# honglu2875/hironaka

Measured on AMD Instinct MI355X. Metric: env-steps/sec at dim=3, max_pts=20, batch=65536; 1/2/4/8 GPUs, higher is better.
Workload: dtype f32

## Files before the change

hironaka_amd/csrc/hk_duo_kernel.h:

```cpp
#pragma once

#include "hk_fast_kernel.h"

namespace hk {

constexpr int kDuoGames = kWave / 2;

__device__ __forceinline__ int duo_other_i(int v) { return qperm_i<0xB1>(v); }
__device__ __forceinline__ float duo_other(float v) { return __int_as_float(duo_other_i(__float_as_int(v))); }

__device__ __forceinline__ uint64_t duo_ballot(bool p) { return __builtin_amdgcn_ballot_w64(p); }

template <int M, int D>
struct DuoGeom {
  using G = FastGeom<M, D>;
  static constexpr int CH = (G::C + 1) / 2;
  static constexpr int QH = (kDuoGames * G::Q + kWave - 1) / kWave;
  static constexpr bool kLean = CH * D <= 30;
};

template <int M, int D>
struct DuoSlabRegs {
  typename VecOf<FastGeom<M, D>::W>::type v[DuoGeom<M, D>::QH];
};

template <int M, int D, bool CONTIG>
__device__ __forceinline__ void duo_slab_issue_impl(DuoSlabRegs<M, D>& r, const float* base, int64_t in_stride,
                                                    int ngames, int lane) {
  using G = FastGeom<M, D>;
  using V = typename VecOf<G::W>::type;
  const int total = ngames * G::Q;
#pragma unroll
  for (int it = 0; it < DuoGeom<M, D>::QH; ++it) {
    int q = lane + it * kWave;
    q = q < total ? q : total - 1;
    r.v[it] = *reinterpret_cast<const V*>(base + slab_chunk_global<M, D, CONTIG>(q, in_stride));
  }
}

template <int M, int D>
__device__ __forceinline__ void duo_slab_issue(DuoSlabRegs<M, D>& r, const float* in, int64_t in_stride, int64_t g0,
                                               int ngames, int lane) {
  const float* base = in + g0 * in_stride;
  if (in_stride == FastGeom<M, D>::N) duo_slab_issue_impl<M, D, true>(r, base, in_stride, ngames, lane);
  else duo_slab_issue_impl<M, D, false>(r, base, in_stride, ngames, lane);
}

template <int M, int D>
__device__ __forceinline__ void duo_slab_commit(DuoSlabRegs<M, D>& r, float* lds, int ngames, int lane) {
  using G = FastGeom<M, D>;
  using V = typename VecOf<G::W>::type;
  const int total = ngames * G::Q;
#pragma unroll
  for (int it = 0; it < DuoGeom<M, D>::QH; ++it) asm volatile("" : "+v"(r.v[it]));
#pragma unroll
  for (int it = 0; it < DuoGeom<M, D>::QH; ++it) {
    const int q = lane + it * kWave;
    if (q < total) *reinterpret_cast<V*>(lds + slab_chunk_lds<M, D>(q)) = r.v[it];
  }
}

constexpr int kStorePlain = 0, kStoreNT = 1, kStoreWT = 2;

template <int M, int D, bool CONTIG, int kBatch, int ST = kStorePlain>
__device__ __forceinline__ void duo_store_slab_impl(const float* lds, float* base, int64_t out_stride, int ngames,
                                                    int lane) {
  using G = FastGeom<M, D>;
  using V = typename VecOf<G::W>::type;
  constexpr int QH = DuoGeom<M, D>::QH;
  constexpr bool kWT = ST == kStoreWT && CONTIG && G::W == 4;
  const int total = ngames * G::Q;
#pragma unroll
  for (int i0 = 0; i0 < QH; i0 += kBatch) {
    V v[kBatch];
#pragma unroll
    for (int u = 0; u < kBatch; ++u) {
      int q = lane + (i0 + u) * kWave;
      q = q < kDuoGames * G::Q ? q : kDuoGames * G::Q - 1;
      v[u] = *reinterpret_cast<const V*>(lds + slab_chunk_lds<M, D>(q));
    }
#pragma unroll
    for (int u = 0; u < kBatch; ++u) asm volatile("" : "+v"(v[u]));
    if constexpr (kWT) {
      typedef unsigned int vu4 __attribute__((ext_vector_type(4)));
      const uint64_t b = (uint64_t)base;
      const uint32_t blo = __builtin_amdgcn_readfirstlane((uint32_t)b), bhi = __builtin_amdgcn_readfirstlane((uint32_t)(b >> 32));
      const int bytes = __builtin_amdgcn_readfirstlane(total * G::W * (int)sizeof(float));
      const auto rsrc = __builtin_amdgcn_make_buffer_rsrc((void*)(((uint64_t)bhi << 32) | blo), 0, bytes, 0x00020000);
#pragma unroll
      for (int u = 0; u < kBatch; ++u) {
        const int q = lane + (i0 + u) * kWave;
        if (i0 + u < QH && q < total)
          __builtin_amdgcn_raw_buffer_store_b128(__builtin_bit_cast(vu4, v[u]), rsrc, q * G::W * (int)sizeof(float), 0,
                                                 16);
      }
    } else {
#pragma unroll
      for (int u = 0; u < kBatch; ++u) {
        const int q = lane + (i0 + u) * kWave;
        if (i0 + u < QH && q < total) {
          V* dst = reinterpret_cast<V*>(base + slab_chunk_global<M, D, CONTIG>(q, out_stride));
          if constexpr (ST != kStorePlain) __builtin_nontemporal_store(v[u], dst);
          else *dst = v[u];
        }
      }
    }
  }
}

template <int M, int D, int kBatch = DuoGeom<M, D>::QH, int ST = kStorePlain>
__device__ inline void duo_store_slab(const float* lds, float* out, int64_t out_stride, int64_t g0, int ngames,
                                      int lane) {
  float* base = out + g0 * out_stride;
  if (out_stride == FastGeom<M, D>::N) duo_store_slab_impl<M, D, true, kBatch, ST>(lds, base, out_stride, ngames, lane);
  else duo_store_slab_impl<M, D, false, kBatch, ST>(lds, base, out_stride, ngames, lane);
}

struct DuoLadder {
  static constexpr int next_bucket(int nb) { return nb < 6 ? nb + 1 : nb + 2; }
};

template <int M, int CH, int D, int SB = CH>
__device__ __forceinline__ void duo_gather_slots(float (&q)[CH * D], const float* mine, uint32_t mask, int smax, int h) {
  mask = h ? (mask & (mask - 1)) : mask;
  unrolled_while<0, SB>([&](auto sc) {
    constexpr int s = decltype(sc)::value;
    if (s >= smax) return false;
    const bool has = mask != 0;
    const float* row = mine + (has ? mask_first(mask) : 0) * D;
    mask &= mask - 1;
    mask &= mask - 1;
#pragma unroll
    for (int k = 0; k < D; ++k) {
      const float v = row[k];
      q[s * D + k] = has ? v : INFINITY;
    }
    return true;
  });
}

template <int CH, int D, int NB, int SB = NB>
__device__ __forceinline__ void duo_gather_level(float (&q)[CH * D], const float* mine, const float* hole, uint32_t mask,
                                                 int h) {
  mask = h ? (mask & (mask - 1)) : mask;
  const float* row[NB];
#pragma unroll
  for (int s = 0; s < NB; ++s) {
    row[s] = mask != 0 ? mine + mask_first(mask) * D : hole;
    mask &= mask - 1;
    mask &= mask - 1;
  }
#pragma unroll
  for (int s = 0; s < NB; ++s)
#pragma unroll
    for (int k = 0; k < D; ++k) q[s * D + k] = row[s][k];
#pragma unroll
  for (int e = NB * D; e < SB * D; ++e) q[e] = INFINITY;
}

template <int M, int CH, int D, bool LEVELS, int SB = CH>
__device__ __forceinline__ void duo_gather(float (&q)[CH * D], const float* mine, const float* hole, uint32_t mask,
                                           int smax, int h) {
  if constexpr (LEVELS) {
    StagesFor<DuoLadder, SB>::run(smax, [&](auto nb) {
      duo_gather_level<CH, D, decltype(nb)::value, SB>(q, mine, hole, mask, h);
      return 0;
    });
  } else {
    duo_gather_slots<M, CH, D, SB>(q, mine, mask, smax, h);
  }
}

template <int CH, int D, int NB>
__device__ __forceinline__ uint32_t duo_scatter_level(const float (&q)[CH * D], float* mine, uint32_t mask, int h) {
  mask = h ? (mask & (mask - 1)) : mask;
  uint32_t alive = 0;
#pragma unroll
  for (int s = 0; s < NB; ++s) {
    if (mask != 0 && q[s * D] < INFINITY) {
      const int slot = mask_first(mask);
      alive |= 1u << slot;
      float* row = mine + slot * D;
#pragma unroll
      for (int k = 0; k < D; ++k) row[k] = q[s * D + k];
    }
    mask &= mask - 1;
    mask &= mask - 1;
  }
  return alive;
}

template <int M, int CH, int D, int SB = CH>
__device__ __forceinline__ uint32_t duo_scatter(const float (&q)[CH * D], float* mine, uint32_t mask, int smax, int h) {
  mask = h ? (mask & (mask - 1)) : mask;
  uint32_t alive = 0;
  unrolled_while<0, SB>([&](auto sc) {
    constexpr int s = decltype(sc)::value;
    if (s >= smax) return false;
    if (mask != 0 && q[s * D] < INFINITY) {
      const int slot = mask_first(mask);
      alive |= 1u << slot;
      float* row = mine + slot * D;
#pragma unroll
      for (int k = 0; k < D; ++k) row[k] = q[s * D + k];
    }
    mask &= mask - 1;
    mask &= mask - 1;
    return true;
  });
  return lanes_or<2>(alive);
}

template <int D>
__device__ __forceinline__ void duo_pad_rows(float* mine, uint32_t dead, float pad, int h) {
  dead = h ? (dead & (dead - 1)) : dead;
  while (dead != 0) {
    float* row = mine + mask_first(dead) * D;
#pragma unroll
    for (int k = 0; k < D; ++k) row[k] = pad;
    dead &= dead - 1;
    dead &= dead - 1;
  }
}

template <int M, int D>
__device__ __forceinline__ void duo_scan_half(const float* mine, float fill, int h, uint32_t& live, bool& ok) {
  static_assert(M <= 32, "the game's mask is one word");
  constexpr int C = (M + 1) / 2;
  const int i0 = h * C;
  const float* base = mine + i0 * D;
  uint32_t mask = 0;
  ok = true;
  const uint32_t fill_bits = __float_as_uint(fill);
#pragma unroll
  for (int r = 0; r < C; ++r) {
    const bool valid = (M % 2 == 0) || r + 1 < C || h == 0;
    uint32_t hi = __float_as_uint(base[r * D]), lo = hi;
#pragma unroll
    for (int k = 1; k < D; ++k) {
      const uint32_t u = __float_as_uint(base[r * D + k]);
      hi = u > hi ? u : hi;
      lo = u < lo ? u : lo;
    }
    const bool ge = hi < 0x7F800000u;
    const bool fl = (lo == fill_bits) && (hi == fill_bits);
    ok &= (ge | fl | !valid);
    mask |= (ge && valid) ? (1u << r) : 0u;
  }
  mask <<= i0;
  live = lanes_or<2>(mask);
}

template <int CH, int D, int NB>
__device__ __forceinline__ void d_newton(float (&q)[CH * D], int h) {
  float acc[NB], oth[NB];
#pragma unroll
  for (int i = 0; i + 1 < NB; ++i) {
#pragma unroll
    for (int j = i + 1; j < NB; ++j) {
      float t, u;
      diff_extrema<D>(&q[i * D], &q[j * D], t, u);
      const float vi = (t > 0.0f) ? -u : 1.0f;
      acc[j] = (i == 0) ? t : hk_fmin(acc[j], t);
      acc[i] = (i == 0 && j == 1) ? vi : hk_fmin(acc[i], vi);
    }
    __builtin_amdgcn_sched_barrier(0);
  }
  const bool late = h != 0;
#pragma unroll
  for (int b = 0; b < NB; ++b) {
    float o[D];
#pragma unroll
    for (int k = 0; k < D; ++k) o[k] = duo_other(q[b * D + k]);
    {
      float t, u;
      diff_extrema<D>(&q[b * D], o, t, u);
      const float va = (t > 0.0f || late) ? -u : 1.0f;
      acc[b] = (NB == 1) ? va : hk_fmin(acc[b], va);
      oth[b] = (u < 0.0f || !late) ? t : 1.0f;
    }
#pragma unroll
    for (int a = 0; a < b; ++a) {
      float t, u;
      diff_extrema<D>(&q[a * D], o, t, u);
      oth[b] = hk_fmin(oth[b], t);
      acc[a] = hk_fmin(acc[a], (t > 0.0f) ? -u : 1.0f);
    }
    __builtin_amdgcn_sched_barrier(0);
  }
#pragma unroll
  for (int r = 0; r < NB; ++r) {
    const bool r0 = acc[r] <= 0.0f, r1 = duo_other(oth[r]) <= 0.0f;
    const bool removed = r0 || r1;
#pragma unroll
    for (int k = 0; k < D; ++k) q[r * D + k] = removed ? INFINITY : q[r * D + k];
  }
}

template <int CH, int D, int NB>
__device__ __forceinline__ void d_shift_words(float (&q)[CH * D], uint32_t cmask, int axis, int np, unsigned flags) {
  bool apply = true;
  if (flags & HK_FLAG_AXIS_NOOP_IF_INVALID) apply = axis >= 0 && ((cmask >> axis) & 1u);
  if ((flags & HK_FLAG_IGNORE_ENDED) && np < 2) apply = false;
  const uint32_t onehot = apply ? 1u << (axis & 31) : 0u;
  uint32_t isax[D], in[D];
#pragma unroll
  for (int k = 0; k < D; ++k) {
    isax[k] = (uint32_t)((int32_t)(onehot << (31 - k)) >> 31);
    in[k] = (uint32_t)((int32_t)(cmask << (31 - k)) >> 31);
    asm volatile("" : "+v"(isax[k]), "+v"(in[k]));
  }
#pragma unroll
  for (int r = 0; r < NB; ++r) {
    float s = __uint_as_float(__float_as_uint(q[r * D]) & in[0]);
#pragma unroll
    for (int k = 1; k < D; ++k) s = s + __uint_as_float(__float_as_uint(q[r * D + k]) & in[k]);
#pragma unroll
    for (int k = 0; k < D; ++k)
      q[r * D + k] = __uint_as_float((__float_as_uint(s) & isax[k]) | (__float_as_uint(q[r * D + k]) & ~isax[k]));
  }
}

template <int CH, int D, int NB, bool BIN = false, bool WORDS = false>
__device__ __forceinline__ int d_stages(float (&q)[CH * D], const float (&c)[D], int axis, int np, int h,
                                        unsigned flags, unsigned stages, uint32_t cmask = 0) {
  static_assert(!WORDS || BIN, "the subset as bits");
  if (stages & HK_STAGE_SHIFT) {
    if constexpr (WORDS) d_shift_words<CH, D, NB>(q, cmask, axis, np, flags);
    else if constexpr (BIN) b_shift_mask<CH, D, NB>(q, cmask, axis, np, flags);
    else b_shift<CH, D, NB>(q, c, axis, np, flags);
  }
  if (stages & HK_STAGE_REPOSITION) reposition<2, CH, D, NB, BIN>(q, flags);
  if (stages & HK_STAGE_NEWTON) d_newton<CH, D, NB>(q, h);
// ... 127 lines not shown
    o.hi = (uint32_t)duo_other_i((int)best.hi);
    o.lo = (uint32_t)duo_other_i((int)best.lo);
    if constexpr (KEEP) {
#pragma unroll
      for (int k = 0; k < D; ++k) o.bd[k] = duo_other(best.bd[k]);
    }
    zeil_merge<D, KEEP>(best, o);
  }
  const bool have = best.have();
  if constexpr (!KEEP) {
    const int i = have ? (int)((best.lo & 0xFFFFu) >> 6) : 0, j = have ? (int)(best.lo & 63u) : 0;
#pragma unroll
    for (int k = 0; k < D; ++k) best.bd[k] = mine[i * D + k] - mine[j * D + k];
    __syncthreads();
  }
  int lo = 0, hi = 0;
  float vlo = best.bd[0], vhi = best.bd[0];
#pragma unroll
  for (int k = 1; k < D; ++k) {
    if (best.bd[k] < vlo) { vlo = best.bd[k]; lo = k; }
    if (best.bd[k] > vhi) { vhi = best.bd[k]; hi = k; }
  }
  if (!have || lo == hi) return 0;
  return encode_mask((1u << lo) | (1u << hi));
}

constexpr int kDuoPreBlocks = 6;

template <int D>
__device__ __forceinline__ void duo_policy_fill(uint8_t* act, uint64_t gg, uint32_t wb0, int nb, uint64_t seed,
                                                int host_policy, int agent_policy, int gi, int h) {
  static_assert(D <= 5 && D <= kPolicyShortDim, "an action travels as a byte; four steps per Philox block");
  auto put = [&](const U4& r, int b) {
    int cls, axis;
    uint32_t mask;
#pragma unroll
    for (int k = 0; k < 4; ++k) {
      const uint32_t w = u4_word(r, k);
      policy_from_words<D>(w & 0xFFFF0000u, w << 16, host_policy, agent_policy, cls, axis, mask, 0);
      act[(4 * b + k) * kDuoGames + gi] = (uint8_t)(mask | ((uint32_t)axis << 5));
    }
  };
#pragma nounroll
  for (int i = 0; i < kDuoPreBlocks; i += 4) {
    if (i >= nb) break;
    const int b0 = i + h, b1 = b0 + 2;
    if (i + 2 < nb) {
      const U4 r0 = philox4x32((uint32_t)gg, (uint32_t)(gg >> 32), wb0 + (uint32_t)b0, kStreamPolicy, seed);
      const U4 r1 = philox4x32((uint32_t)gg, (uint32_t)(gg >> 32), wb0 + (uint32_t)b1, kStreamPolicy, seed);
      put(r0, b0);
      if (b1 < kDuoPreBlocks) put(r1, b1);
    } else {
      const U4 r0 = philox4x32((uint32_t)gg, (uint32_t)(gg >> 32), wb0 + (uint32_t)b0, kStreamPolicy, seed);
      if (b0 < kDuoPreBlocks) put(r0, b0);
    }
  }
}

template <int M, int D, int MODE, int HOT = kHotNone, bool ACTS = false, bool ZEIL = false>
__global__ __launch_bounds__(kWave, 2) void duo_kernel(const float* in0, int64_t in_stride0, int batch0,
                                                       const Params prm) {
  static_assert(!ACTS || MODE == kModeRollout, "the small records ride on the plain rollout");
  static_assert(!ZEIL || (MODE == kModeRollout && HOT == kHotNone && !ACTS), "Zeillinger's host: plain rollouts");
  constexpr bool kRec = MODE == kModeRolloutRec;
  constexpr bool kRoll = MODE == kModeRollout || kRec;
  constexpr bool kPartialPublish = MODE == kModeRollout && !ZEIL && DuoGeom<M, D>::kLean;
  constexpr bool kLevelDeal = MODE == kModeRollout && DuoGeom<M, D>::kLean;
  using G = FastGeom<M, D>;
  constexpr int CH = DuoGeom<M, D>::CH;
  static_assert(M <= 32, "the live mask of a game travels as 32 bits");
  __shared__ __align__(16) float lds[kDuoGames * G::S];
  __shared__ float cbuf[kDuoGames * D];
  __shared__ float hole_row[D];
  __shared__ __align__(16) uint8_t pol[(MODE == kModeRollout) ? (4 * kDuoPreBlocks + 1) * kDuoGames : 16];
  const int lane = threadIdx.x;
  const int h = lane & 1, gi = lane >> 1;
  const int64_t g0 = (int64_t)blockIdx.x * kDuoGames;
  const int64_t left = (int64_t)batch0 - g0;
  const int ngames = (int)(left < kDuoGames ? left : kDuoGames);
  const bool active = gi < ngames;
  const bool leader = active && h == 0;
  const int64_t g = g0 + gi;
#ifdef HK_DUO_PROBE
  __shared__ int32_t probe_buf[24];
  if (lane < 24) probe_buf[lane] = 0;
  const long long probe_t0 = wall_clock64();
  long long probe_t1 = 0, probe_t2 = 0;
  int probe_steps = 0, probe_smax = 0;
#endif
  const bool has_ids = kRoll && prm.game_ids != nullptr;
  uint32_t raw_id = 0;
  if (has_ids && active) raw_id = (uint32_t)prm.game_ids[g];
  __builtin_amdgcn_sched_barrier(0);
  DuoSlabRegs<M, D> slab;
  duo_slab_issue<M, D>(slab, in0, in_stride0, g0, ngames, lane);
  __builtin_amdgcn_sched_barrier(0);
  const uint64_t gg = prm.game_offset + (has_ids ? (uint64_t)raw_id : (uint64_t)g);
  uint32_t pol_b0 = prm.step_offset >> 2;
  const uint32_t pol_last = (prm.steps > 0) ? (prm.step_offset + (uint32_t)prm.steps - 1u) >> 2 : pol_b0;
  if constexpr (MODE == kModeRollout && !ZEIL) {
    const uint32_t nb = pol_last - pol_b0 + 1u;
    duo_policy_fill<D>(pol, gg, pol_b0, (int)(nb < (uint32_t)kDuoPreBlocks ? nb : (uint32_t)kDuoPreBlocks), prm.seed,
                       HOT ? (int)HK_HOST_RANDOM : prm.host_policy,
                       (HOT == kHotJax) ? (int)HK_AGENT_RANDOM
                                        : (HOT == kHotTorch) ? (int)HK_AGENT_RANDOM_LEGAL : prm.agent_policy, gi, h);
  }
#ifdef HK_DUO_PROBE
  if (lane == 0) probe_buf[21] = (int32_t)wall_clock64();
#endif
  float* mine = lds + gi * G::S;
  const float pad = (float)prm.pad;
  const unsigned flags = (HOT == kHotJax) ? (unsigned)HK_SEM_JAX : (HOT == kHotTorch) ? kHotTorchFlags : prm.flags;
  const unsigned stages = HOT ? (unsigned)(HK_STAGE_SHIFT | HK_STAGE_REPOSITION | HK_STAGE_NEWTON) : prm.stages;
  const float fill = ((flags & HK_SEM_MASK) == HK_SEM_JAX) ? -1.0f : pad;
  const int nsteps = kRoll ? prm.steps : 1;
  constexpr bool kEndSort = MODE == kModeRollout && HOT == kHotNone;
  const bool end_sort = kEndSort && nsteps > 0 && (stages & HK_STAGE_NEWTON) &&
                        ((flags & HK_SEM_MASK) == HK_SEM_LIST || (flags & HK_FLAG_COMPACT_SORTED));
  bool rescale_pending = false;
  PolicyCache pcache;
  DuoPolicyCache dcache;
  float c[D];
  int axis_in = -1;
#pragma unroll
  for (int k = 0; k < D; ++k) c[k] = 0.0f;
  RawActions<D> raw;
  const bool fetch_actions = !kRoll && (stages & HK_STAGE_SHIFT) && active;
  if (fetch_actions) fast_fetch_actions<D>(prm, g, M, raw);
  duo_slab_commit<M, D>(slab, lds, ngames, lane);
  if (kLevelDeal && lane < D) hole_row[lane] = INFINITY;
  if (fetch_actions) fast_decode_actions<D>(prm, raw, c, axis_in);
  __syncthreads();
#ifdef HK_DUO_PROBE
  if (lane == 0) probe_buf[22] = (int32_t)wall_clock64();
#endif

  uint32_t gmask;
  bool ok;
  duo_scan_half<M, D>(mine, fill, h, gmask, ok);
  if (!active) {
    gmask = 0;
    ok = true;
  }
  int np = mask_pop(gmask);
  int nmax = wave_max(np, M);
  const bool exact = (fill == pad) && __all(ok) && nmax <= G::C;

  if (!exact) {
    float* cs = cbuf + gi * D;
    np = leader ? num_points<float>(mine, M, D) : 2;
    int length = (np < 2) ? 0 : -1;
    if (kRoll && prm.count_ws) {
      const unsigned long long b0 = __ballot(leader && np < 2);
      if (lane == 0) count_add(prm.count_ws + blockIdx.x, (uint32_t)__popcll(b0));
    }
    for (int t = 0; t < nsteps; ++t) {
      int axis = axis_in, cls = 0;
      if (kRec && prm.obs_out) {
        __syncthreads();
        duo_store_slab<M, D, 2>(lds, (float*)prm.obs_out + (int64_t)t * prm.batch * G::N, (int64_t)G::N, g0, ngames, lane);
        __syncthreads();
      }
      if (kRoll) {
        uint32_t mask;
        const int zc = (prm.host_policy == HK_HOST_ZEILLINGER && leader) ? zeillinger_game<float>(mine, prm.m, prm.d) : 0;
        fast_policy<D>(prm, gg, prm.step_offset + (uint32_t)t, pcache, cls, axis, mask, zc);
        if (leader)
          for (int k = 0; k < prm.d; ++k) cs[k] = (float)((mask >> k) & 1u);
      } else if ((stages & HK_STAGE_SHIFT) && leader) {
        load_coords<float>(prm, g, cs);
      }
      const bool prev_done = np < 2;
      if (leader) {
        stages_game<float>(mine, prm.m, prm.d, cs, axis, pad, stages, flags);
        np = num_points<float>(mine, prm.m, prm.d);
      }
      const bool done = np < 2;
      if (done && length < 0) length = t + 1;
      if (kRoll && prm.count_ws) {
        const unsigned long long bd = __ballot(leader && done);
        if (lane == 0) count_add(prm.count_ws + (size_t)(t + 1) * prm.count_stride + blockIdx.x, (uint32_t)__popcll(bd));
      }
      if ((kRec || ACTS) && leader) {
        const int64_t at = (int64_t)t * prm.batch + g;
        if (prm.r_host_class_out) prm.r_host_class_out[at] = cls;
        if (prm.r_axis_out) prm.r_axis_out[at] = axis;
        if (prm.r_done_out) prm.r_done_out[at] = done;
        if (prm.r_reward_out) prm.r_reward_out[at] = prm.reward_sign * (float)(done && !prev_done);
      }
      if (!kRoll && leader) {
        if (prm.done_out) prm.done_out[g] = done;
        if (prm.prev_done_out) prm.prev_done_out[g] = prev_done;
        if (prm.reward_out) prm.reward_out[g] = prm.reward_sign * (float)(done && !prev_done);
        if (prm.num_points_out) prm.num_points_out[g] = np;
      }
    }
    if (kRoll && leader && prm.game_length_out) prm.game_length_out[g] = length;
    __syncthreads();
    duo_store_slab<M, D>(lds, (float*)prm.out, prm.out_stride, g0, ngames, lane);
    return;
  }

  if (kPartialPublish && h == 0) reinterpret_cast<uint32_t*>(cbuf)[gi] = gmask;
  int smax = (nmax + 1) >> 1;
#ifdef HK_DUO_PROBE
  probe_t1 = wall_clock64();
  probe_smax = smax;
#endif
  float q[CH * D];
  if constexpr (!kLevelDeal) {
#pragma unroll
    for (int e = 0; e < CH * D; ++e) q[e] = INFINITY;
  }
  duo_gather<M, CH, D, kLevelDeal>(q, mine, hole_row, gmask, smax, h);
#ifdef HK_DUO_PROBE
  {
    float sink = 0.0f;
#pragma unroll
    for (int e = 0; e < CH * D; ++e) sink += (q[e] < INFINITY) ? q[e] : 0.0f;
    asm volatile("" : "+v"(sink));
    if (lane == 0) probe_buf[23] = (int32_t)wall_clock64();
  }
#endif
  if (!active) np = 2;
  int length = (np < 2) ? 0 : -1;
  if (kRoll && prm.count_ws) {
    const unsigned long long b0 = __ballot(leader && np < 2);
    if (lane == 0) count_add(prm.count_ws + blockIdx.x, (uint32_t)__popcll(b0));
// ... 44 lines not shown
  };
  if constexpr (MODE == kModeRollout) {
    static_assert(CH <= 6 || CH % 2 == 0, "bucket ladder: 1..6, then even numbers");
    uint64_t amask = duo_ballot(active), lmask = duo_ballot(leader);
    asm volatile("" : "+s"(amask), "+s"(lmask));
    int open_steps = (np < 2) ? -1 : 0;
    auto length_at = [&](int tt) { return open_steps == tt ? -1 : open_steps + 1; };
    int t = 0;
    bool stop = false;
    while (t < nsteps && !stop) {
    if (!ZEIL && (uint32_t)((step0 + (uint32_t)t) >> 2) - pol_b0 >= (uint32_t)kDuoPreBlocks) {
      if constexpr (want_small) {
        length = length_at(t);
        flush_records(__builtin_amdgcn_readfirstlane(t));
      }
      __syncthreads();
      pol_b0 = (step0 + (uint32_t)t) >> 2;
      const uint32_t nb = pol_last - pol_b0 + 1u;
      duo_policy_fill<D>(pol, gg, pol_b0, (int)(nb < (uint32_t)kDuoPreBlocks ? nb : (uint32_t)kDuoPreBlocks), seed,
                         host_policy, agent_policy, gi, h);
      __syncthreads();
    }
    const uint32_t wend_abs = (pol_b0 + (uint32_t)kDuoPreBlocks) << 2;
    const int tw = (!ZEIL && wend_abs - step0 < (uint32_t)nsteps) ? (int)(wend_abs - step0) : nsteps;
    uint32_t a_next = ZEIL ? 0u : pol[(int)(step0 + (uint32_t)t - (pol_b0 << 2)) * kDuoGames + gi];
    Levels<DuoLadder, CH>::run([&](auto nbc, auto loc) {
      constexpr int NB = decltype(nbc)::value, LO = decltype(loc)::value;
      if (!((smax > LO || LO == 0) && t < tw && !stop)) return;
#ifndef HK_NO_SETPRIO
      if (t >= 10) __builtin_amdgcn_s_setprio(3);
      else if constexpr (NB >= 6) __builtin_amdgcn_s_setprio(3);
      else if constexpr (NB >= 4) __builtin_amdgcn_s_setprio(2);
      else if constexpr (NB >= 2) __builtin_amdgcn_s_setprio(1);
      else __builtin_amdgcn_s_setprio(0);
#endif
      auto play = [&](int tend) {
        while (t < tend) {
          uint32_t mask;
          int axis;
          if constexpr (ZEIL) {
            static_assert(NB <= kDuoZeilDpp || 2 * NB <= M, "the rolled pair loop parks ranks 0 .. 2 NB - 1 in the game's M rows");
            const int zc = (duo_ballot(np >= 2) & amask) != 0 ? duo_zeillinger<CH, D, NB>(q, h, mine, smax) : 0;
            uint32_t ra, rb;
            int cls;
            duo_policy_words(gg, step0 + (uint32_t)t, seed, dcache, h, ra, rb);
            policy_from_words<D>(ra, rb, host_policy, agent_policy, cls, axis, mask, zc);
          } else {
            const uint32_t a = a_next;
            a_next = pol[(int)(step0 + (uint32_t)t + 1u - (pol_b0 << 2)) * kDuoGames + gi];
            mask = a & 31u;
            axis = (int)(a >> 5);
          }
          const unsigned st = (end_sort && t + 1 == nsteps) ? (stages & ~(unsigned)HK_STAGE_RESCALE) : stages;
          rescale_pending = end_sort && t + 1 == nsteps && (stages & HK_STAGE_RESCALE);
          const int np_new = d_stages<CH, D, NB, true, (NB == 1)>(q, c, axis, np, h, flags, st, mask);
#ifdef HK_DUO_PROBE
          if (lane == 0 && t == 0) probe_buf[20] = (int32_t)wall_clock64();
#endif
          if constexpr (NB == 1) {
            const uint64_t live = duo_ballot(q[0] < INFINITY);
            const uint64_t open = live & (live >> 1) & lmask;
            open_steps += __builtin_amdgcn_inverse_ballot_w64(open) ? 1 : 0;
            np = __builtin_amdgcn_inverse_ballot_w64(open | (open << 1)) ? 2 : 0;
            if (open == 0) {
              uint32_t any_bits = __float_as_uint(q[0]);
#pragma unroll
              for (int k = 1; k < D; ++k) any_bits |= __float_as_uint(q[k]);
              if ((duo_ballot(any_bits != 0u) & live & amask) == 0) {
                stop = true;
                tend = 0;
              }
            }
          } else {
            np = np_new;
            open_steps += (leader && np >= 2) ? 1 : 0;
            if ((duo_ballot(np >= 2 * smax - 1) & amask) == 0) {
              int left = nsteps - 1 - t;
              asm volatile("" : "+s"(left));
              if (left > 0) {
                __syncthreads();
                if constexpr (kLevelDeal) {
                  gmask = lanes_or<2>(duo_scatter_level<CH, D, NB>(q, mine, gmask, h));
                  __syncthreads();
                  nmax = wave_max(active ? np : 0, 2 * smax - 2);
                  smax = (nmax + 1) >> 1;
                  duo_gather_level<CH, D, NB>(q, mine, hole_row, gmask, h);
                } else {
                  gmask = duo_scatter<M, CH, D, NB>(q, mine, gmask, smax, h);
                  __syncthreads();
                  const int sprev = smax;
                  nmax = wave_max(active ? np : 0, 2 * smax - 2);
                  smax = (nmax + 1) >> 1;
                  duo_gather_slots<M, CH, D, NB>(q, mine, gmask, sprev, h);
                }
                tend = smax <= LO ? 0 : tend;
              }
            }
          }
#ifdef HK_DUO_PROBE
          if (lane == 0 && t < 24) probe_buf[t] = (int32_t)((((uint32_t)wall_clock64()) << 4) | (uint32_t)(smax & 15));
#endif
          ++t;
        }
      };
      if constexpr (NB == 1) {
        play(tw < 10 ? tw : 10);
        if (t < tw && !stop) {
#ifndef HK_NO_SETPRIO
          __builtin_amdgcn_s_setprio(3);
#endif
          play(tw);
        }
      } else {
        play(tw);
      }
    });
    }
    length = length_at(t);
#ifdef HK_DUO_PROBE
    probe_steps = t;
    probe_t2 = wall_clock64();
#endif
    if (count_slot) add_length_counts(count_slot, count_stride, 1, nsteps, leader, length, lane);
    if constexpr (want_small) {
      for (;;) {
        const uint32_t wend = ((pol_b0 + (uint32_t)kDuoPreBlocks) << 2) - step0;
        const int te = __builtin_amdgcn_readfirstlane((wend < (uint32_t)nsteps) ? (int)wend : nsteps);
        flush_records(te);
        if (te >= nsteps) break;
        __syncthreads();
        pol_b0 = (step0 + (uint32_t)te) >> 2;
        const uint32_t nb = pol_last - pol_b0 + 1u;
        duo_policy_fill<D>(pol, gg, pol_b0, (int)(nb < (uint32_t)kDuoPreBlocks ? nb : (uint32_t)kDuoPreBlocks), seed,
                           host_policy, agent_policy, gi, h);
        __syncthreads();
      }
    }
  }
  const bool want_obs = kRec && prm.obs_out != nullptr;
  const bool want_records = kRec && (prm.r_host_class_out || prm.r_axis_out || prm.r_done_out || prm.r_reward_out);
  for (int t = 0; MODE != kModeRollout && t < nsteps; ++t) {
    int axis = axis_in, cls = 0;
    if (want_obs) {
      __syncthreads();
      if (h == 0) fill_image<M, D>(mine, pad);
      __syncthreads();
      duo_scatter<M, CH, D>(q, mine, gmask, smax, h);
      __syncthreads();
      duo_store_slab<M, D, 2>(lds, (float*)prm.obs_out + (int64_t)t * prm.batch * G::N, (int64_t)G::N, g0, ngames, lane);
    }
    uint32_t mask = 0;
    if (kRoll) {
      uint32_t ra, rb;
      duo_policy_words(gg, step0 + (uint32_t)t, seed, dcache, h, ra, rb);
      policy_from_words<D>(ra, rb, host_policy, agent_policy, cls, axis, mask, 0);
    }
    const bool prev_done = np < 2;
    const unsigned st = (end_sort && t + 1 == nsteps) ? (stages & ~(unsigned)HK_STAGE_RESCALE) : stages;
    rescale_pending = end_sort && t + 1 == nsteps && (stages & HK_STAGE_RESCALE);
    np = DuoStagesFor<CH, D, 1, kRoll>::run(q, smax, c, axis, np, h, flags, st, mask);
    if (!active) np = 2;
    const bool done = np < 2;
    if (done && length < 0) length = t + 1;
    if (!kRoll && leader) {
      if (prm.done_out) prm.done_out[g] = done;
      if (prm.prev_done_out) prm.prev_done_out[g] = prev_done;
      if (prm.reward_out) prm.reward_out[g] = prm.reward_sign * (float)(done && !prev_done);
      if (prm.num_points_out) prm.num_points_out[g] = np;
    }
    if (want_records && leader) {
      const int64_t at = (int64_t)t * prm.batch + g;
      if (prm.r_host_class_out) prm.r_host_class_out[at] = cls;
      if (prm.r_axis_out) prm.r_axis_out[at] = axis;
      if (prm.r_done_out) prm.r_done_out[at] = done;
      if (prm.r_reward_out) prm.r_reward_out[at] = prm.reward_sign * (float)(done && !prev_done);
    }
    const unsigned long long bd = __ballot(leader && done);
    if (count_slot && lane == 0) count_add(count_slot + (size_t)(t + 1) * count_stride, (uint32_t)__popcll(bd));
    if (MODE == kModeRollout && smax == 1 && bd == __ballot(leader) && t + 1 < nsteps) {
      bool still = true;
#pragma unroll
      for (int k = 0; k < D; ++k) still &= (q[k] == 0.0f);
      still |= !(q[0] < INFINITY);
      if (!__any(active && !still)) {
        if (count_slot && lane == 0)
          for (int tt = t + 1; tt < nsteps; ++tt) count_add(count_slot + (size_t)(tt + 1) * count_stride, (uint32_t)__popcll(bd));
        break;
      }
    }
    if (t + 1 < nsteps && !__any(active && ((np + 1) >> 1) >= smax)) {
      __syncthreads();
      gmask = duo_scatter<M, CH, D>(q, mine, gmask, smax, h);
      __syncthreads();
      const int sprev = smax;
      nmax = wave_max(active ? np : 0, 2 * smax - 2);
      smax = (nmax + 1) >> 1;
      duo_gather_slots<M, CH, D>(q, mine, gmask, sprev, h);
    }
  }
  if (kRoll && leader && prm.game_length_out) prm.game_length_out[g] = length;

  __syncthreads();
  if (kPartialPublish && !end_sort) {
    const uint32_t alive = duo_scatter<M, CH, D>(q, mine, gmask, smax, h);
    duo_pad_rows<D>(mine, reinterpret_cast<const uint32_t*>(cbuf)[gi] & ~alive, pad, h);
  } else {
    if (h == 0) fill_image<M, D>(mine, pad);
    __syncthreads();
    if (kEndSort && end_sort) {
      int rank[CH];
      duo_ranks_first<CH, D>(q, smax, rank);
      if (rescale_pending) rescale<2, CH, D, CH>(q, flags);
      duo_scatter_ranked<CH, D>(q, mine, rank, smax);
    } else {
      duo_scatter<M, CH, D>(q, mine, gmask, smax, h);
    }
  }
  __syncthreads();
  constexpr int kFinalStore = MODE != kModeRollout ? kStorePlain : DuoGeom<M, D>::kLean ? kStoreWT : kStoreNT;
  duo_store_slab<M, D, DuoGeom<M, D>::QH, kFinalStore>(lds, (float*)prm.out, prm.out_stride, g0, ngames, lane);
#ifdef HK_DUO_PROBE
  if (kRoll && lane == 0 && prm.game_length_out && ngames >= 8) {
    int32_t* w = prm.game_length_out + g0;
    w[0] = (int32_t)probe_t0;
    w[1] = (int32_t)probe_t1;
    w[2] = (int32_t)probe_t2;
    w[3] = (int32_t)wall_clock64();
    w[4] = probe_steps;
    w[5] = probe_smax;
    w[6] = (int32_t)blockIdx.x;
    w[7] = (int32_t)__builtin_amdgcn_s_getreg((4 << 0) | (0 << 6) | (31 << 11));
    if (ngames >= 32)
      for (int i = 0; i < 24; ++i) w[8 + i] = probe_buf[i];
  }
#endif
}

inline int device_simds() {
  static int cached[16] = {0};
  int dev = 0;
  if (hipGetDevice(&dev) != hipSuccess || dev < 0 || dev >= 16) dev = 0;
  if (!cached[dev]) {
    int cus = 0;
    if (hipDeviceGetAttribute(&cus, hipDeviceAttributeMultiprocessorCount, dev) != hipSuccess || cus <= 0) cus = 256;
    (void)hipGetLastError();
    cached[dev] = 4 * cus;
  }
  return cached[dev];
}

inline bool duo_supported(const Params& prm, int dtype) {
  if ((prm.mode != kModeRollout && prm.mode != kModeStep) || prm.m > 32) return false;
  if (prm.mode == kModeStep && (prm.class_out || (prm.stages & kStageFeatureSorts))) return false;
  if (prm.mode == kModeRollout && prm.host_policy == HK_HOST_ZEILLINGER && any_records(prm)) return false;
  if (sorted_output(prm) && (prm.mode != kModeRollout || any_records(prm))) return false;
  return fast_supported(prm, dtype);
}

template <int M, int D>
int launch_duo_t(Params prm, hipStream_t stream) {
  const unsigned grid = (unsigned)(((int64_t)prm.batch + kDuoGames - 1) / kDuoGames);
  prm.games_per_block = kDuoGames;
  launch_prepare();
  const bool records = prm.obs_out != nullptr;
  const bool acts = small_records_only(prm);
  const int hot = (prm.mode == kModeRollout && !records) ? fast_hot_config(prm) : kHotNone;
  if (prm.mode == kModeRollout && records)
    hipLaunchKernelGGL((duo_kernel<M, D, kModeRolloutRec>), dim3(grid), dim3(kWave), 0, stream, (const float*)prm.in,
                       prm.in_stride, prm.batch, prm);
  else if (prm.mode == kModeRollout && prm.host_policy == HK_HOST_ZEILLINGER)
    hipLaunchKernelGGL((duo_kernel<M, D, kModeRollout, kHotNone, false, true>), dim3(grid), dim3(kWave), 0, stream,
                       (const float*)prm.in, prm.in_stride, prm.batch, prm);
  else if (prm.mode == kModeRollout && acts && hot == kHotJax)
    hipLaunchKernelGGL((duo_kernel<M, D, kModeRollout, kHotJax, true>), dim3(grid), dim3(kWave), 0, stream,
                       (const float*)prm.in, prm.in_stride, prm.batch, prm);
  else if (prm.mode == kModeRollout && acts)
    hipLaunchKernelGGL((duo_kernel<M, D, kModeRollout, kHotNone, true>), dim3(grid), dim3(kWave), 0, stream,
                       (const float*)prm.in, prm.in_stride, prm.batch, prm);
  else if (prm.mode == kModeStep && prm.flags == HK_SEM_JAX &&
           prm.stages == (HK_STAGE_SHIFT | HK_STAGE_REPOSITION | HK_STAGE_NEWTON))
    hipLaunchKernelGGL((duo_kernel<M, D, kModeStep, kHotJax>), dim3(grid), dim3(kWave), 0, stream,
                       (const float*)prm.in, prm.in_stride, prm.batch, prm);
  else if (prm.mode == kModeStep)
    hipLaunchKernelGGL((duo_kernel<M, D, kModeStep>), dim3(grid), dim3(kWave), 0, stream, (const float*)prm.in,
                       prm.in_stride, prm.batch, prm);
  else if (hot == kHotJax)
    hipLaunchKernelGGL((duo_kernel<M, D, kModeRollout, kHotJax>), dim3(grid), dim3(kWave), 0, stream,
                       (const float*)prm.in, prm.in_stride, prm.batch, prm);
  else if (hot == kHotTorch)
    hipLaunchKernelGGL((duo_kernel<M, D, kModeRollout, kHotTorch>), dim3(grid), dim3(kWave), 0, stream,
                       (const float*)prm.in, prm.in_stride, prm.batch, prm);
  else
    hipLaunchKernelGGL((duo_kernel<M, D, kModeRollout>), dim3(grid), dim3(kWave), 0, stream, (const float*)prm.in,
                       prm.in_stride, prm.batch, prm);
  return launch_status();
}

#ifndef HK_SPEC_TU
#define HK_X(M_, D_) extern template int launch_duo_t<M_, D_>(Params, hipStream_t);
HK_FAST_SPECS(HK_X)
#undef HK_X

inline int launch_duo(const Params& prm, hipStream_t stream) {
#define HK_X(M_, D_) if (prm.m == M_ && prm.d == D_) return launch_duo_t<M_, D_>(prm, stream);
  HK_FAST_SPECS(HK_X)
#undef HK_X
  return HK_ERR_UNSUPPORTED;
}
#endif

}
```

hironaka_amd/csrc/hk_duo_spec.hip:

```cpp
#define HK_SPEC_TU 1
#include "hk_duo_kernel.h"

namespace hk {
static_assert(HK_SPEC_M * HK_SPEC_D > 0, "build with -DHK_SPEC_M=<max_points> -DHK_SPEC_D=<dim>");
template int launch_duo_t<HK_SPEC_M, HK_SPEC_D>(Params, hipStream_t);
}
```

hironaka_amd/csrc/hk_quad_kernel.h:

```cpp
#pragma once

#include "hk_fast_kernel.h"

namespace hk {

constexpr int kQuad = 4;
constexpr int kQuadGames = kWave / kQuad;

constexpr int kQuadUp1 = 0x39, kQuadUp2 = 0x4E, kQuadUp3 = 0x93;

template <int M, int D>
struct QuadGeom {
  static constexpr int N = M * D;
  static constexpr int W = (N % 4 == 0) ? 4 : ((N % 2 == 0) ? 2 : 1);
  static constexpr int Q = N / W;
  static constexpr int QL = (kQuadGames * Q + kWave - 1) / kWave;
  static constexpr int R = (M + kQuad - 1) / kQuad;
  static constexpr bool kBig = N * kQuadGames * 4 > 8 * 1024;
  static constexpr int CW = kBig ? ((D <= 4) ? 4 : D) : ((D <= 3) ? 4 : D + 1);
  static constexpr int kImage = kQuadGames * N;
  static constexpr int kCompact = kBig ? 0 : kQuadGames * M * CW;
  static constexpr int kRegion = kBig ? kQuadGames * (N > M * CW ? N : M * CW) : kImage + kCompact;
  static constexpr int kGameStride = kBig ? (N > M * CW ? N : M * CW) : N;
  static constexpr int kStoreBatch = QL < 12 ? QL : 10;
  static constexpr int kLdsPerGroup = 4 * (kRegion * 4 + kQuadGames * D * 4);
  static constexpr int kWavesPerSimd = kBig ? 2 : ((160 * 1024 / kLdsPerGroup) < 4 ? (160 * 1024 / kLdsPerGroup) : 4);
  static constexpr int next_bucket(int nb) { return nb < 6 ? nb + 1 : (nb < 10 ? nb + 2 : nb + 3); }
  static_assert(!kBig || kGameStride == N, "the aliased layout assumes the compact rows fit the image");
};

constexpr int kDmaImm = 4096;
template <int BYTES, int OFFSET>
__device__ __forceinline__ void lds_dma(const float* src, float* dst) {
  static_assert(BYTES == 16 || BYTES == 4, "request size");
  if constexpr (BYTES == 16) __builtin_amdgcn_global_load_lds(src, dst, 16, OFFSET, 0);
  else __builtin_amdgcn_global_load_lds(src, dst, 4, OFFSET, 0);
}

template <int M, int D>
__device__ __forceinline__ void quad_slab_load(const float* base, float* image, int ngames, int lane) {
  using G = QuadGeom<M, D>;
  constexpr int CH = (G::W == 4) ? 4 : 1;
  constexpr int FULL = kQuadGames * G::N / CH;
  constexpr int QF = (FULL + kWave - 1) / kWave;
  const float* src = base + (unsigned)lane * CH;
  const unsigned total = (unsigned)ngames * (G::N / CH);
  if (ngames == kQuadGames) {
    unrolled_while<0, QF>([&](auto ic) {
      constexpr int it = decltype(ic)::value;
      if ((it + 1) * kWave <= FULL || lane < FULL - it * kWave)
        lds_dma<CH * 4, (it * kWave * CH * 4) % kDmaImm>(src + (it * kWave * CH * 4) / kDmaImm * (kDmaImm / 4),
                                                        image + (it * kWave * CH * 4) / kDmaImm * (kDmaImm / 4));
      return true;
    });
  } else {
    unrolled_while<0, QF>([&](auto ic) {
      constexpr int it = decltype(ic)::value;
      if ((unsigned)lane + it * kWave < total)
        lds_dma<CH * 4, (it * kWave * CH * 4) % kDmaImm>(src + (it * kWave * CH * 4) / kDmaImm * (kDmaImm / 4),
                                                        image + (it * kWave * CH * 4) / kDmaImm * (kDmaImm / 4));
      return true;
    });
  }
}

__device__ __forceinline__ void wait_vmem_all() { __builtin_amdgcn_s_waitcnt(0x0F70); }

template <int M, int D, bool NT = false>
__device__ __forceinline__ void quad_slab_store(const float* image, float* base, int ngames, int lane) {
  using G = QuadGeom<M, D>;
  using V = typename VecOf<G::W>::type;
  constexpr int B = G::kStoreBatch;
  constexpr int FULL = kQuadGames * G::Q;
  const unsigned total = (unsigned)ngames * G::Q;
  const float* src = image + (unsigned)lane * G::W;
  float* dst = base + (unsigned)lane * G::W;
  const bool whole = ngames == kQuadGames;
#pragma unroll
  for (int i0 = 0; i0 < G::QL; i0 += B) {
    V v[B];
#pragma unroll
    for (int u = 0; u < B; ++u) {
      if (i0 + u < G::QL) v[u] = *reinterpret_cast<const V*>(src + (i0 + u) * kWave * G::W);
    }
#pragma unroll
    for (int u = 0; u < B; ++u) asm volatile("" : "+v"(v[u]));
    if (whole) {
#pragma unroll
      for (int u = 0; u < B; ++u) {
        const int it = i0 + u;
        if (it < G::QL && ((it + 1) * kWave <= FULL || lane < FULL - it * kWave)) {
          if constexpr (NT) __builtin_nontemporal_store(v[u], reinterpret_cast<V*>(dst + it * kWave * G::W));
          else *reinterpret_cast<V*>(dst + it * kWave * G::W) = v[u];
        }
      }
    } else {
#pragma unroll
      for (int u = 0; u < B; ++u) {
        const int it = i0 + u;
        if (it < G::QL && (unsigned)lane + it * kWave < total) {
          if constexpr (NT) __builtin_nontemporal_store(v[u], reinterpret_cast<V*>(dst + it * kWave * G::W));
          else *reinterpret_cast<V*>(dst + it * kWave * G::W) = v[u];
        }
      }
    }
  }
}

__device__ __forceinline__ void wave_lds_fence() {
  __builtin_amdgcn_fence(__ATOMIC_RELEASE, "wavefront");
  __builtin_amdgcn_wave_barrier();
  __builtin_amdgcn_fence(__ATOMIC_ACQUIRE, "wavefront");
}

template <int R, int D, int NB>
__device__ __forceinline__ void qd_rescale(float (&q)[R * D], unsigned flags) {
  const bool jax_sem = (flags & HK_SEM_MASK) == HK_SEM_JAX;
  float mx = -1.0f;
#pragma unroll
  for (int r = 0; r < NB; ++r) {
    const bool live = q[r * D] < INFINITY;
#pragma unroll
    for (int k = 0; k < D; ++k) mx = hk_fmax(mx, live ? q[r * D + k] : -1.0f);
  }
  mx = lanes_max<kQuad>(mx);
  const bool skip = jax_sem ? (mx <= 1e-8f) : (mx < 0.0f);
  const float div = (skip || mx == 0.0f) ? 1.0f : mx;
#pragma unroll
  for (int r = 0; r < NB; ++r) {
    const bool live = q[r * D] < INFINITY;
#pragma unroll
    for (int k = 0; k < D; ++k) q[r * D + k] = live ? q[r * D + k] / div : INFINITY;
    __builtin_amdgcn_sched_barrier(0);
  }
}

template <int D, int ORDER, bool ACC_FIRST = false, bool OTH_FIRST = false>
__device__ __forceinline__ void qd_pair(const float* mine, const float* other, float& acc, float& oth, bool late) {
  float t, u;
  diff_extrema<D>(mine, other, t, u);
  float vo, va;
  if (ORDER > 0) {
    vo = t;
    va = (t > 0.0f) ? -u : 1.0f;
  } else if (ORDER < 0) {
    vo = (u < 0.0f) ? t : 1.0f;
    va = -u;
  } else {
    vo = (u < 0.0f || !late) ? t : 1.0f;
// ... 1285 lines not shown
```

Baseline: 62.76 billion.

## Load duo slab via global-to-LDS DMA, cheaper scan validity check, DPP wave max

For contiguous, aligned inputs with no game ids, the duo kernel now loads the input slab straight into LDS with global_load_lds, skipping the register staging and commit. The scan's per-row validity check becomes a single OR-accumulated bitwise difference, and the wave-wide max reduction uses DPP row operations for lean geometries. The LDS DMA helpers move into a shared header, and optional probe timing instrumentation is added. The DMA path drains all vector memory before use, which gives up any overlap between the slab load and the action fetch.

```diff
diff --git a/hironaka_amd/csrc/hk_duo_kernel.h b/hironaka_amd/csrc/hk_duo_kernel.h
--- a/hironaka_amd/csrc/hk_duo_kernel.h
+++ b/hironaka_amd/csrc/hk_duo_kernel.h
@@ -1,10 +1,25 @@
 #pragma once
 
 #include "hk_fast_kernel.h"
+#include "hk_lds_dma.h"
 
 namespace hk {
 
 constexpr int kDuoGames = kWave / 2;
+
+#ifndef HK_DUO_LEGS
+#define HK_DUO_LEGS 3
+#endif
+#ifdef HK_DUO_PROBE
+constexpr int kDuoProbeRow = 48, kDuoProbeWaves = 4096;
+static __device__ int32_t duo_probe_rows[kDuoProbeWaves * kDuoProbeRow];
+#define HK_DUO_PROBE_PARAM , int32_t* probe = nullptr
+#define HK_DUO_PROBE_ARG(p) , p
+#else
+#define HK_DUO_PROBE_PARAM
+#define HK_DUO_PROBE_ARG(p)
+#endif
+constexpr bool kDuoLegDma = (HK_DUO_LEGS & 1) != 0, kDuoLegScan = (HK_DUO_LEGS & 2) != 0;
 
 __device__ __forceinline__ int duo_other_i(int v) { return qperm_i<0xB1>(v); }
 __device__ __forceinline__ float duo_other(float v) { return __int_as_float(duo_other_i(__float_as_int(v))); }
@@ -60,11 +75,45 @@
   }
 }
 
+template <int M, int D>
+struct DuoDma {
+  using G = FastGeom<M, D>;
+  static constexpr bool kShape = kDuoLegDma && G::W == 4 && G::S == G::N;
+};
+
+template <int M, int D>
+__device__ __forceinline__ void duo_slab_dma(const float* base, float* image, int ngames, int lane) {
+  using G = FastGeom<M, D>;
+  constexpr int FULL = kDuoGames * G::Q;
+  constexpr int QH = DuoGeom<M, D>::QH;
+  constexpr int kImm = kDmaImm;
+  static_assert(DuoDma<M, D>::kShape, "the image is the slab");
+  const float* src = base + (unsigned)lane * 4;
+  const unsigned total = (unsigned)ngames * G::Q;
+  if (ngames == kDuoGames) {
+    unrolled_while<0, QH>([&](auto ic) {
+      constexpr int it = decltype(ic)::value;
+      if ((it + 1) * kWave <= FULL || lane < FULL - it * kWave)
+        lds_dma<16, (it * kWave * 16) % kImm>(src + (it * kWave * 16) / kImm * (kImm / 4),
+                                             image + (it * kWave * 16) / kImm * (kImm / 4));
+      return true;
+    });
+  } else {
+    unrolled_while<0, QH>([&](auto ic) {
+      constexpr int it = decltype(ic)::value;
+      if ((unsigned)lane + it * kWave < total)
+        lds_dma<16, (it * kWave * 16) % kImm>(src + (it * kWave * 16) / kImm * (kImm / 4),
+                                             image + (it * kWave * 16) / kImm * (kImm / 4));
+      return true;
+    });
+  }
+}
+
 constexpr int kStorePlain = 0, kStoreNT = 1, kStoreWT = 2;
 
 template <int M, int D, bool CONTIG, int kBatch, int ST = kStorePlain>
 __device__ __forceinline__ void duo_store_slab_impl(const float* lds, float* base, int64_t out_stride, int ngames,
-                                                    int lane) {
+                                                    int lane HK_DUO_PROBE_PARAM) {
   using G = FastGeom<M, D>;
   using V = typename VecOf<G::W>::type;
   constexpr int QH = DuoGeom<M, D>::QH;
@@ -81,6 +130,9 @@
     }
 #pragma unroll
     for (int u = 0; u < kBatch; ++u) asm volatile("" : "+v"(v[u]));
+#ifdef HK_DUO_PROBE
+    if (probe && lane == 0) probe[0] = (int32_t)wall_clock64();
+#endif
     if constexpr (kWT) {
       typedef unsigned int vu4 __attribute__((ext_vector_type(4)));
       const uint64_t b = (uint64_t)base;
@@ -110,10 +162,13 @@
 
 template <int M, int D, int kBatch = DuoGeom<M, D>::QH, int ST = kStorePlain>
 __device__ inline void duo_store_slab(const float* lds, float* out, int64_t out_stride, int64_t g0, int ngames,
-                                      int lane) {
+                                      int lane HK_DUO_PROBE_PARAM) {
   float* base = out + g0 * out_stride;
-  if (out_stride == FastGeom<M, D>::N) duo_store_slab_impl<M, D, true, kBatch, ST>(lds, base, out_stride, ngames, lane);
-  else duo_store_slab_impl<M, D, false, kBatch, ST>(lds, base, out_stride, ngames, lane);
+  if (out_stride == FastGeom<M, D>::N) duo_store_slab_impl<M, D, true, kBatch, ST>(lds, base, out_stride, ngames, lane HK_DUO_PROBE_ARG(probe));
+  else duo_store_slab_impl<M, D, false, kBatch, ST>(lds, base, out_stride, ngames, lane HK_DUO_PROBE_ARG(probe));
+#ifdef HK_DUO_PROBE
+  if (probe && lane == 0) probe[1] = (int32_t)wall_clock64();
+#endif
 }
 
 struct DuoLadder {
@@ -230,8 +285,9 @@
   const int i0 = h * C;
   const float* base = mine + i0 * D;
   uint32_t mask = 0;
-  ok = true;
   const uint32_t fill_bits = __float_as_uint(fill);
+  uint32_t off = 0;
+  bool okb = true;
 #pragma unroll
   for (int r = 0; r < C; ++r) {
     const bool valid = (M % 2 == 0) || r + 1 < C || h == 0;
@@ -243,12 +299,31 @@
       lo = u < lo ? u : lo;
     }
     const bool ge = hi < 0x7F800000u;
-    const bool fl = (lo == fill_bits) && (hi == fill_bits);
-    ok &= (ge | fl | !valid);
+    if constexpr (DuoGeom<M, D>::kLean && kDuoLegScan) {
+      const uint32_t differs = (hi ^ fill_bits) | (lo ^ fill_bits);
+      off |= (ge || !valid) ? 0u : differs;
+    } else {
+      const bool fl = (lo == fill_bits) && (hi == fill_bits);
+      okb &= (ge | fl | !valid);
+    }
     mask |= (ge && valid) ? (1u << r) : 0u;
   }
+  ok = (DuoGeom<M, D>::kLean && kDuoLegScan) ? off == 0u : okb;
   mask <<= i0;
   live = lanes_or<2>(mask);
+}
+
+template <bool DPP>
+__device__ __forceinline__ int duo_wave_max(int v, int hi) {
+  if constexpr (!DPP) return wave_max(v, hi);
+  auto mx = [](int a, int b) { return a > b ? a : b; };
+  v = mx(v, __builtin_amdgcn_update_dpp(0, v, 0x111, 0xF, 0xF, true));
+  v = mx(v, __builtin_amdgcn_update_dpp(0, v, 0x112, 0xF, 0xF, true));
+  v = mx(v, __builtin_amdgcn_update_dpp(0, v, 0x114, 0xF, 0xF, true));
+  v = mx(v, __builtin_amdgcn_update_dpp(0, v, 0x118, 0xF, 0xF, true));
+  v = mx(v, __builtin_amdgcn_update_dpp(0, v, 0x142, 0xA, 0xF, false));
+  v = mx(v, __builtin_amdgcn_update_dpp(0, v, 0x143, 0xC, 0xF, false));
+  return __builtin_amdgcn_readlane(v, kWave - 1);
 }
 
 template <int CH, int D, int NB>
@@ -542,20 +617,39 @@
   const bool leader = active && h == 0;
   const int64_t g = g0 + gi;
 #ifdef HK_DUO_PROBE
-  __shared__ int32_t probe_buf[24];
-  if (lane < 24) probe_buf[lane] = 0;
+  __shared__ int32_t probe_buf[32];
+  if (lane < 32) probe_buf[lane] = 0;
   const long long probe_t0 = wall_clock64();
   long long probe_t1 = 0, probe_t2 = 0;
   int probe_steps = 0, probe_smax = 0;
 #endif
   const bool has_ids = kRoll && prm.game_ids != nullptr;
   uint32_t raw_id = 0;
-  if (has_ids && active) raw_id = (uint32_t)prm.game_ids[g];
-  __builtin_amdgcn_sched_barrier(0);
   DuoSlabRegs<M, D> slab;
-  duo_slab_issue<M, D>(slab, in0, in_stride0, g0, ngames, lane);
-  __builtin_amdgcn_sched_barrier(0);
-  const uint64_t gg = prm.game_offset + (has_ids ? (uint64_t)raw_id : (uint64_t)g);
+  uint64_t gg;
+  bool dma = false;
+  if constexpr (DuoDma<M, D>::kShape) {
+    if (has_ids) {
+      if (active) raw_id = (uint32_t)prm.game_ids[g];
+      __builtin_amdgcn_sched_barrier(0);
+      duo_slab_issue<M, D>(slab, in0, in_stride0, g0, ngames, lane);
+      __builtin_amdgcn_sched_barrier(0);
+      asm volatile("" : "+v"(raw_id));
+      gg = prm.game_offset + (uint64_t)raw_id;
+    } else {
+      dma = in_stride0 == G::N && ((uintptr_t)in0 & 15u) == 0;
+      if (dma) duo_slab_dma<M, D>(in0 + g0 * G::N, lds, ngames, lane);
+      else duo_slab_issue<M, D>(slab, in0, in_stride0, g0, ngames, lane);
+      __builtin_amdgcn_sched_barrier(0);
+      gg = prm.game_offset + (uint64_t)g;
+    }
+  } else {
+    if (has_ids && active) raw_id = (uint32_t)prm.game_ids[g];
+    __builtin_amdgcn_sched_barrier(0);
+    duo_slab_issue<M, D>(slab, in0, in_stride0, g0, ngames, lane);
+    __builtin_amdgcn_sched_barrier(0);
+    gg = prm.game_offset + (has_ids ? (uint64_t)raw_id : (uint64_t)g);
+  }
   uint32_t pol_b0 = prm.step_offset >> 2;
   const uint32_t pol_last = (prm.steps > 0) ? (prm.step_offset + (uint32_t)prm.steps - 1u) >> 2 : pol_b0;
   if constexpr (MODE == kModeRollout && !ZEIL) {
@@ -587,7 +681,12 @@
   RawActions<D> raw;
   const bool fetch_actions = !kRoll && (stages & HK_STAGE_SHIFT) && active;
   if (fetch_actions) fast_fetch_actions<D>(prm, g, M, raw);
-  duo_slab_commit<M, D>(slab, lds, ngames, lane);
+  if constexpr (DuoDma<M, D>::kShape) {
+    if (dma) wait_vmem_all();
+    else duo_slab_commit<M, D>(slab, lds, ngames, lane);
+  } else {
+    duo_slab_commit<M, D>(slab, lds, ngames, lane);
+  }
   if (kLevelDeal && lane < D) hole_row[lane] = INFINITY;
   if (fetch_actions) fast_decode_actions<D>(prm, raw, c, axis_in);
   __syncthreads();
@@ -603,7 +702,11 @@
     ok = true;
   }
   int np = mask_pop(gmask);
-  int nmax = wave_max(np, M);
+#ifdef HK_DUO_PROBE
+  asm volatile("" : "+v"(np));
+  if (lane == 0) probe_buf[24] = (int32_t)wall_clock64();
+#endif
+  int nmax = duo_wave_max<DuoGeom<M, D>::kLean && kDuoLegScan>(np, M);
   const bool exact = (fill == pad) && __all(ok) && nmax <= G::C;
 
   if (!exact) {
@@ -814,14 +917,14 @@
                 if constexpr (kLevelDeal) {
                   gmask = lanes_or<2>(duo_scatter_level<CH, D, NB>(q, mine, gmask, h));
                   __syncthreads();
-                  nmax = wave_max(active ? np : 0, 2 * smax - 2);
+                  nmax = duo_wave_max<DuoGeom<M, D>::kLean && kDuoLegScan>(active ? np : 0, 2 * smax - 2);
                   smax = (nmax + 1) >> 1;
                   duo_gather_level<CH, D, NB>(q, mine, hole_row, gmask, h);
                 } else {
                   gmask = duo_scatter<M, CH, D, NB>(q, mine, gmask, smax, h);
                   __syncthreads();
                   const int sprev = smax;
-                  nmax = wave_max(active ? np : 0, 2 * smax - 2);
+                  nmax = duo_wave_max<DuoGeom<M, D>::kLean && kDuoLegScan>(active ? np : 0, 2 * smax - 2);
                   smax = (nmax + 1) >> 1;
                   duo_gather_slots<M, CH, D, NB>(q, mine, gmask, sprev, h);
                 }
@@ -925,12 +1028,15 @@
       gmask = duo_scatter<M, CH, D>(q, mine, gmask, smax, h);
       __syncthreads();
       const int sprev = smax;
-      nmax = wave_max(active ? np : 0, 2 * smax - 2);
+      nmax = duo_wave_max<DuoGeom<M, D>::kLean && kDuoLegScan>(active ? np : 0, 2 * smax - 2);
       smax = (nmax + 1) >> 1;
       duo_gather_slots<M, CH, D>(q, mine, gmask, sprev, h);
     }
   }
   if (kRoll && leader && prm.game_length_out) prm.game_length_out[g] = length;
+#ifdef HK_DUO_PROBE
+  if (lane == 0) probe_buf[25] = (int32_t)wall_clock64();
+#endif
 
   __syncthreads();
   if (kPartialPublish && !end_sort) {
@@ -949,11 +1055,15 @@
     }
   }
   __syncthreads();
+#ifdef HK_DUO_PROBE
+  if (lane == 0) probe_buf[26] = (int32_t)wall_clock64();
+#endif
   constexpr int kFinalStore = MODE != kModeRollout ? kStorePlain : DuoGeom<M, D>::kLean ? kStoreWT : kStoreNT;
-  duo_store_slab<M, D, DuoGeom<M, D>::QH, kFinalStore>(lds, (float*)prm.out, prm.out_stride, g0, ngames, lane);
-#ifdef HK_DUO_PROBE
-  if (kRoll && lane == 0 && prm.game_length_out && ngames >= 8) {
-    int32_t* w = prm.game_length_out + g0;
+  duo_store_slab<M, D, DuoGeom<M, D>::QH, kFinalStore>(lds, (float*)prm.out, prm.out_stride, g0, ngames,
+                                                       lane HK_DUO_PROBE_ARG(probe_buf + 27));
+#ifdef HK_DUO_PROBE
+  if (kRoll && lane == 0 && blockIdx.x < (unsigned)kDuoProbeWaves) {
+    int32_t* w = duo_probe_rows + blockIdx.x * kDuoProbeRow;
     w[0] = (int32_t)probe_t0;
     w[1] = (int32_t)probe_t1;
     w[2] = (int32_t)probe_t2;
@@ -962,8 +1072,7 @@
     w[5] = probe_smax;
     w[6] = (int32_t)blockIdx.x;
     w[7] = (int32_t)__builtin_amdgcn_s_getreg((4 << 0) | (0 << 6) | (31 << 11));
-    if (ngames >= 32)
-      for (int i = 0; i < 24; ++i) w[8 + i] = probe_buf[i];
+    for (int i = 0; i < 32; ++i) w[8 + i] = probe_buf[i];
   }
 #endif
 }
diff --git a/hironaka_amd/csrc/hk_duo_spec.hip b/hironaka_amd/csrc/hk_duo_spec.hip
--- a/hironaka_amd/csrc/hk_duo_spec.hip
+++ b/hironaka_amd/csrc/hk_duo_spec.hip
@@ -5,3 +5,11 @@
 static_assert(HK_SPEC_M * HK_SPEC_D > 0, "build with -DHK_SPEC_M=<max_points> -DHK_SPEC_D=<dim>");
 template int launch_duo_t<HK_SPEC_M, HK_SPEC_D>(Params, hipStream_t);
 }
+
+#ifdef HK_DUO_PROBE
+extern "C" int hk_duo_probe_read(int32_t* dst, int waves) {
+  if (waves < 0 || waves > hk::kDuoProbeWaves) return -1;
+  return (int)hipMemcpyFromSymbol(dst, HIP_SYMBOL(hk::duo_probe_rows), (size_t)waves * hk::kDuoProbeRow * sizeof(int32_t), 0,
+                                  hipMemcpyDeviceToHost);
+}
+#endif
diff --git a/hironaka_amd/csrc/hk_lds_dma.h b/hironaka_amd/csrc/hk_lds_dma.h
--- /dev/null
+++ b/hironaka_amd/csrc/hk_lds_dma.h
@@ -0,0 +1,15 @@
+#pragma once
+
+namespace hk {
+
+constexpr int kDmaImm = 4096;
+template <int BYTES, int OFFSET>
+__device__ __forceinline__ void lds_dma(const float* src, float* dst) {
+  static_assert(BYTES == 16 || BYTES == 4, "request size");
+  if constexpr (BYTES == 16) __builtin_amdgcn_global_load_lds(src, dst, 16, OFFSET, 0);
+  else __builtin_amdgcn_global_load_lds(src, dst, 4, OFFSET, 0);
+}
+
+__device__ __forceinline__ void wait_vmem_all() { __builtin_amdgcn_s_waitcnt(0x0F70); }
+
+}
diff --git a/hironaka_amd/csrc/hk_quad_kernel.h b/hironaka_amd/csrc/hk_quad_kernel.h
--- a/hironaka_amd/csrc/hk_quad_kernel.h
+++ b/hironaka_amd/csrc/hk_quad_kernel.h
@@ -1,6 +1,7 @@
 #pragma once
 
 #include "hk_fast_kernel.h"
+#include "hk_lds_dma.h"
 
 namespace hk {
 
@@ -28,14 +29,6 @@
   static constexpr int next_bucket(int nb) { return nb < 6 ? nb + 1 : (nb < 10 ? nb + 2 : nb + 3); }
   static_assert(!kBig || kGameStride == N, "the aliased layout assumes the compact rows fit the image");
 };
-
-constexpr int kDmaImm = 4096;
-template <int BYTES, int OFFSET>
-__device__ __forceinline__ void lds_dma(const float* src, float* dst) {
-  static_assert(BYTES == 16 || BYTES == 4, "request size");
-  if constexpr (BYTES == 16) __builtin_amdgcn_global_load_lds(src, dst, 16, OFFSET, 0);
-  else __builtin_amdgcn_global_load_lds(src, dst, 4, OFFSET, 0);
-}
 
 template <int M, int D>
 __device__ __forceinline__ void quad_slab_load(const float* base, float* image, int ngames, int lane) {
@@ -63,8 +56,6 @@
     });
   }
 }
-
-__device__ __forceinline__ void wait_vmem_all() { __builtin_amdgcn_s_waitcnt(0x0F70); }
 
 template <int M, int D, bool NT = false>
 __device__ __forceinline__ void quad_slab_store(const float* image, float* base, int ngames, int lane) {
```

Result: faster. 64.36 billion (median of 6 runs) (+2.5%).
